# gorse-io/gorse

Measured on AMD Instinct MI355X. Metric: BPR positive-samples/sec (whole job, N GPUs), higher is better.
Workload: dtype f32; 1 GPU; S-ml1m 6040x3706x994169 per rank (C2), nFactors=64; factors_finite=True

## Files before the change

### gorse_amd/csrc/bpr.hip

```cpp
#include <algorithm>
#include <cstdlib>
#include <cstring>

#include "bpr_bins.hpp"
#include "mf_internal.hpp"
#include <utility>

using namespace gorse;

namespace {

int g_variant = 0;
constexpr int MODE_ATOMIC = GORSE_BPR_HOGWILD_ATOMIC;
constexpr int MODE_EXACT = GORSE_BPR_SEQUENTIAL;
constexpr int MODE_RACY = GORSE_BPR_HOGWILD_RACY;
constexpr int MODE_STORES = GORSE_BPR_HOGWILD_STORES;

__global__ __launch_bounds__(256) void bpr_sample_kernel(int32_t U, int32_t I, const int64_t *__restrict__ uptr,
                                                         const int32_t *__restrict__ uidx,
                                                         const int32_t *__restrict__ usorted, uint64_t seed,
                                                         uint64_t epoch, int64_t sample_base, int64_t n,
                                                         int32_t *__restrict__ us, int32_t *__restrict__ is,
                                                         int32_t *__restrict__ js, int32_t *__restrict__ fail_count) {
    for (int64_t s = (int64_t)blockIdx.x * blockDim.x + threadIdx.x; s < n; s += (int64_t)gridDim.x * blockDim.x) {
// ... 549 lines not shown
        }
        __syncthreads();
        if (!big) {
            for (int k = wid; k < ub; k += kFinThreads / 64) {
                const int32_t beg = k ? cnt[k - 1] : 0, len = cnt[k] - beg;
                const uint32_t salt = group_salt(ulo + k);
                if (group && len >= 3 && len <= kGroupCap && ulo + k < U) wave_sort_run(key + beg, len, lane);
                for (int t = lane; t < len; t += 64) {
                    const int2 v = group_unkey(key[beg + t], salt);
                    key[beg + t] = ((uint64_t)(uint32_t)v.y << 32) | (uint32_t)v.x;
                }
            }
            __syncthreads();
        }
        for (int p = tid; p < ms; p += kFinThreads) {
            si[b0 + s0 + p] = (int32_t)(uint32_t)key[p];
            sj[b0 + s0 + p] = (int32_t)(key[p] >> 32);
        }
        __syncthreads();
    }
    if (tid == 0 && nfail > 0) atomicAdd(fail_count, nfail);
    if (big && group)
        for (int k = 0; k < ub && ulo + k < U; k++) {
            const int32_t beg = k ? cnt[k - 1] : 0, len = cnt[k] - beg;
            if (len >= 3 && len <= kGroupCap) group_run<kFinThreads>(key, b0 + beg, len, group_salt(ulo + k), si, sj);
        }
}

template <int MODE>
__device__ __forceinline__ float load_row(const float *p) {
    if (MODE == MODE_EXACT)
        return *p;
    else
        return __hip_atomic_load(p, __ATOMIC_RELAXED, __HIP_MEMORY_SCOPE_AGENT);
}
template <int MODE>
__device__ __forceinline__ void apply(float *p, float snap, float t, float lr, bool fused) {
    if constexpr (MODE == MODE_ATOMIC) {
        (void)snap;
        (void)fused;
        __hip_atomic_fetch_add(p, t * lr, __ATOMIC_RELAXED, __HIP_MEMORY_SCOPE_AGENT);
    } else {
        float r = fused ? fmaf(t, lr, snap) : t * lr + snap;
        if constexpr (MODE == MODE_EXACT)
            *p = r;
        else
            __hip_atomic_store(p, r, __ATOMIC_RELAXED, __HIP_MEMORY_SCOPE_AGENT);
    }
}

__device__ __forceinline__ float bpr_exp(float x, int exp_mode) {
    return exp_mode == 1 ? exp_restated(x) : (exp_mode == 2 ? __expf(x) : expf(x));
}

template <int MODE>
__device__ __forceinline__ void update_elem(float *pu, float *qi, float *qj, int e, float p, float a, float b, float grad,
                                            float nreg, float lr, bool fused, bool same_item) {
    float t1 = p * grad;
    t1 = fused ? fmaf(a, nreg, t1) : a * nreg + t1;
    float t2 = p * (-grad);
    t2 = fused ? fmaf(b, nreg, t2) : b * nreg + t2;
    float t3 = a - b;
    t3 = t3 * grad;
    t3 = fused ? fmaf(p, nreg, t3) : p * nreg + t3;
    if constexpr (MODE == MODE_EXACT) {
        float qi_new = fused ? fmaf(t1, lr, a) : t1 * lr + a;
        qi[e] = qi_new;
        float base = same_item ? qi_new : b;
        qj[e] = fused ? fmaf(t2, lr, base) : t2 * lr + base;
        pu[e] = fused ? fmaf(t3, lr, p) : t3 * lr + p;
    } else {
        apply<MODE>(qi + e, a, t1, lr, fused);
        apply<MODE>(qj + e, b, t2, lr, fused);
        apply<MODE>(pu + e, p, t3, lr, fused);
    }
}

constexpr int kHotReplicas = GORSE_HOT_REPLICAS;
constexpr int kFolderBlocks = 32;
constexpr int kFolderBlocksAcc = 32;
constexpr int kDefaultAccFoldEvery = 4;
int g_acc_fold_every = kDefaultAccFoldEvery;
constexpr uint32_t kDefaultFoldPeriod = 800;
uint32_t g_fold_period = kDefaultFoldPeriod;
constexpr uint64_t kFolderTimeout = 1000000000ull;

struct HotRows {
    const int32_t *slot;
    const int32_t *items;
    const int32_t *meta;
    float *rep;
    int32_t *done;
    int n_hot;
    int d;
    int set;
    uint32_t period;
    int n_acc;
    int acc_every;
};

__device__ __forceinline__ float *hot_row(const HotRows &hot, int32_t code, int64_t group) {
    return hot.rep + (hot_base(code) + (group & ((1 << hot_lg(code)) - 1))) * hot.d;
}

constexpr int kDoneStripes = GORSE_HOT_DONE_STRIPES, kDoneStride = GORSE_HOT_DONE_STRIDE;
constexpr int kFoldPassesWord = 2 * kDoneStripes * kDoneStride;
__device__ __forceinline__ int32_t *done_set(const HotRows &hot, int set) { return hot.done + set * kDoneStripes * kDoneStride; }
template <bool LAST>
__device__ __forceinline__ void worker_done(const HotRows &hot) {
    if constexpr (LAST) asm volatile("s_waitcnt vmcnt(0)" ::: "memory");
    __syncthreads();
    if (threadIdx.x == 0) {
        if constexpr (LAST) {
            __builtin_amdgcn_fence(__ATOMIC_RELEASE, "agent");
            asm volatile("s_waitcnt vmcnt(0)" ::: "memory");
        }
        __hip_atomic_fetch_add(done_set(hot, hot.set) + (blockIdx.x & (kDoneStripes - 1)) * kDoneStride, 1, __ATOMIC_RELAXED,
                               __HIP_MEMORY_SCOPE_AGENT);
    }
}
__device__ __forceinline__ bool workers_done(const HotRows &hot, int workers) {
    const int lane = threadIdx.x & 63;
    const int32_t *c = done_set(hot, hot.set);
    int v = lane < kDoneStripes ? __hip_atomic_load(c + lane * kDoneStride, __ATOMIC_RELAXED, __HIP_MEMORY_SCOPE_AGENT) : 0;
#pragma unroll
    for (int o = 32; o > 0; o >>= 1) v += __shfl_xor(v, o, 64);
    return v >= workers;
}

__device__ __forceinline__ void fold_pass(const HotRows &hot, float *Q, int s0, int s1, int64_t tid, int64_t nthreads) {
    const int d = hot.d;
    const int64_t work = (int64_t)(s1 - s0) * d;
    for (int64_t w = tid; w < work; w += nthreads) {
        const int64_t slot = s0 + w / d;
        const int e = (int)(w - (slot - s0) * d);
        const int32_t code = hot.meta[slot];
        const int nr = 1 << hot_lg(code);
        float *r0 = hot.rep + hot_base(code) * d + e;
        float v[kHotReplicas];
#pragma unroll
        for (int r = 0; r < kHotReplicas; r++)
            v[r] = r < nr ? __hip_atomic_exchange(r0 + (int64_t)r * d, 0.0f, __ATOMIC_RELAXED, __HIP_MEMORY_SCOPE_AGENT) : 0.0f;
        float sum = 0.0f;
#pragma unroll
        for (int r = 0; r < kHotReplicas; r++) sum += v[r];
        if (sum != 0.0f)
            __hip_atomic_fetch_add(Q + (int64_t)hot.items[slot] * d + e, sum, __ATOMIC_RELAXED, __HIP_MEMORY_SCOPE_AGENT);
    }
}

constexpr int kAccBatch = 4;
__device__ __forceinline__ void fold_acc_pass(const HotRows &hot, float *Q, int s0, int s1, int tid, int nthreads) {
    const int d = hot.d;
    const int work = (s1 - s0) * d;
    for (int wb = tid; wb < work; wb += kAccBatch * nthreads) {
        float v[kAccBatch];
        float *q[kAccBatch];
#pragma unroll
        for (int b = 0; b < kAccBatch; b++) {
            const int w = wb + b * nthreads;
            v[b] = 0.0f;
            q[b] = Q;
            if (w < work) {
                const int slot = s0 + w / d;
                const int e = w - (slot - s0) * d;
                q[b] = Q + (int64_t)hot.items[slot] * d + e;
                v[b] = __hip_atomic_exchange(hot.rep + hot_base(hot.meta[slot]) * d + e, 0.0f, __ATOMIC_RELAXED, __HIP_MEMORY_SCOPE_AGENT);
// ... 179 lines not shown
    for (int64_t t0 = 0; t0 < nt; t0 += 256) {
        const int64_t t = t0 + threadIdx.x;
        const int32_t v = t < nt ? sums[t] : 0;
        int32_t total;
        const int32_t ex = block_exclusive_scan_256(v, lds, &total);
        if (t < nt) sums[t] = carry + ex;
        carry += total;
    }
}

__global__ __launch_bounds__(256) void scan_apply_kernel(int32_t *__restrict__ data, int64_t m,
                                                         const int32_t *__restrict__ sums) {
    __shared__ int32_t lds[4];
    const int64_t base = (int64_t)blockIdx.x * kScanTile + (int64_t)threadIdx.x * 8;
    int32_t x[8], v = 0;
#pragma unroll
    for (int e = 0; e < 8; e++) {
        x[e] = base + e < m ? data[base + e] : 0;
        v += x[e];
    }
    int32_t run = sums[blockIdx.x] + block_exclusive_scan_256(v, lds, nullptr);
#pragma unroll
    for (int e = 0; e < 8; e++) {
        if (base + e < m) data[base + e] = run;
        run += x[e];
    }
}


__global__ __launch_bounds__(256) void bpr_scatter_by_kernel(const int32_t *__restrict__ key, const int32_t *__restrict__ us,
                                                             const int32_t *__restrict__ is, const int32_t *__restrict__ js,
                                                             int64_t n, int32_t K, const int32_t *__restrict__ bucket,
                                                             const int32_t *__restrict__ rank, int32_t *__restrict__ su,
                                                             int32_t *__restrict__ si, int32_t *__restrict__ sj) {
    for (int64_t s = (int64_t)blockIdx.x * blockDim.x + threadIdx.x; s < n; s += (int64_t)gridDim.x * blockDim.x) {
        const int32_t kk = key[s] < 0 ? K : key[s];
        const int64_t pos = (int64_t)bucket[kk] + rank[s];
        su[pos] = us[s];
        si[pos] = is[s];
        sj[pos] = js[s];
    }
}

constexpr int kCold = -2;
constexpr int kSeriesFlush = 8;
#ifndef GORSE_BPR_SERIES_SKIP_GATHERS
#define GORSE_BPR_SERIES_SKIP_GATHERS 1
#endif

#ifndef GORSE_BPR_D8_PAIRS
#define GORSE_BPR_D8_PAIRS 1
#endif
template <int NC, bool NEG_STORE, bool D8 = false>
__global__ __launch_bounds__(kBlock) void bpr_update_user_kernel(float *P, float *Q, const int32_t *__restrict__ si,
                                                                 const int32_t *__restrict__ sj,
                                                                 const int32_t *__restrict__ off, int32_t U, int d,
                                                                 float lr, float reg, int exp_mode, double *loss,
                                                                 HotRows hot, int folders, int neg_replicas) {
    if ((int)blockIdx.x < folders) {
        run_folders<true>(hot, Q, folders);
        return;
    }
    auto continues = [](int i0, int j0, int i1, int j1) { return i0 == i1 && (i0 | j0 | j1) >= 0 && i0 != j0 && i0 != j1; };
    const int glane = threadIdx.x & (kGroup - 1);
    const int lane = D8 ? (glane & 7) : glane;
    constexpr int SUBS = D8 && GORSE_BPR_D8_PAIRS ? 2 : 1;
    const bool writer = !D8 || SUBS == 2 || glane < 8;
    auto mad = [](float x, float y, float z) { return D8 ? x * y + z : fmaf(x, y, z); };
    auto tree8 = [](float v) { return SUBS == 2 ? group_tree8_halves(v) : group_tree8(v); };
    const int gib = threadIdx.x / kGroup;
    const int64_t group = ((int64_t)((int)blockIdx.x - folders) * kGroupsPerBlock + gib) * SUBS + (SUBS == 2 ? glane >> 3 : 0);
    const int64_t ngroups = (int64_t)((int)gridDim.x - folders) * kGroupsPerBlock * SUBS;
    const float nreg = -reg;
    double my_loss = 0.0;
    const bool open = folders > 0;
    const bool look_i = open;
    const bool look_j = (open && neg_replicas) || NEG_STORE;
    const int32_t *slot_of = (look_i || look_j) ? hot.slot : si;
    int im1 = -1, jm1 = -1, im2 = -1, jm2 = -1;
    for (int64_t u = group; u < U; u += ngroups) {
        const int beg = off[u], end = off[u + 1];
        if (beg >= end) continue;
        float *pu = P + u * d;
        constexpr int G = 2, IA = 3;
        constexpr int GB = NEG_STORE ? 1 : G;
        float p[NC], ra[G][NC], rb[GB][NC];
        const int last = end - 1;
        auto at = [&](int s) { return s <= last ? s : last; };
        auto cl = [](int x) { return x < 0 ? 0 : x; };
        auto idx_i = [&](int i_, int j_) { return look_i ? cl(i_) : (look_j ? cl(j_) : beg); };
        auto idx_j = [&](int i_, int j_) { return look_j ? cl(j_) : (look_i ? cl(i_) : beg); };
        int ii[IA], jj[IA], sli[G], slj[G];
#pragma unroll
        for (int k = 0; k < IA; k++) ii[k] = si[at(beg + k)], jj[k] = sj[at(beg + k)];
#pragma unroll
        for (int k = 0; k < G; k++) sli[k] = slot_of[idx_i(ii[k], jj[k])], slj[k] = slot_of[idx_j(ii[k], jj[k])];
        float cur[NC], acc[NC];
        bool cont = false;
        int pending = 0;
#pragma unroll
        for (int c = 0; c < NC; c++) {
            p[c] = load_row<MODE_ATOMIC>(pu + 16 * c + lane);
#pragma unroll
            for (int k = 0; k < G; k++) ra[k][c] = load_row<MODE_ATOMIC>(Q + (int64_t)cl(ii[k]) * d + 16 * c + lane);
#pragma unroll
            for (int k = 0; k < GB; k++) rb[k][c] = load_row<MODE_ATOMIC>(Q + (int64_t)cl(jj[k]) * d + 16 * c + lane);
        }
        for (int s = beg; s < end; s++) {
            const int in_ = si[at(s + IA)], jn_ = sj[at(s + IA)];
            const int sli_n = slot_of[idx_i(ii[G], jj[G])];
            const int slj_n = slot_of[idx_j(ii[G], jj[G])];
            const int i = ii[0], j = jj[0], slot = sli[0], slotj = slj[0];
            float(&a)[NC] = ra[0];
            float(&b)[NC] = rb[0];
            float ran[NC], rbn[NC];
            const bool gather_i = !GORSE_BPR_SERIES_SKIP_GATHERS || !(s + G <= last && continues(ii[G - 1], jj[G - 1], ii[G], jj[G]));
#pragma unroll
            for (int c = 0; c < NC; c++) ran[c] = 0.0f;
            if (gather_i) {
#pragma unroll
                for (int c = 0; c < NC; c++) ran[c] = load_row<MODE_ATOMIC>(Q + (int64_t)cl(ii[G]) * d + 16 * c + lane);
            }
#pragma unroll
            for (int c = 0; c < NC; c++) rbn[c] = load_row<MODE_ATOMIC>(Q + (int64_t)cl(jj[GB]) * d + 16 * c + lane);
            if (cont) {
#pragma unroll
                for (int c = 0; c < NC; c++) a[c] = cur[c];
            }
            const bool more = s < last && continues(i, j, ii[1], jj[1]);
            const bool valid = j >= 0;
            float *qi = Q + (int64_t)cl(i) * d, *qj = Q + (int64_t)cl(j) * d;
            if (open && slot >= 0) qi = hot_row(hot, slot, group);
            if (open && neg_replicas && slotj >= 0) qj = hot_row(hot, slotj, group);
            bool st_j = false;
            if constexpr (NEG_STORE) {
                const bool own_j = i == j || j == im1 || j == jm1 || j == im2 || j == jm2;
                st_j = slotj == kCold && !own_j;
            }
            const float diff = D8 ? tree8(p[0] * a[0]) - tree8(p[0] * b[0]) : dot512_regs<NC>(p, a) - dot512_regs<NC>(p, b);
            const float ex = bpr_exp(-diff, exp_mode);
            const float grad = ex / (1.0f + ex);
            if (loss && (SUBS == 2 ? (glane & 7) == 0 : glane == 0) && valid) my_loss += (double)log1pf(ex);
            float t1[NC], t2[NC];
#pragma unroll
            for (int c = 0; c < NC; c++) {
                t1[c] = mad(a[c], nreg, p[c] * grad);
                t2[c] = mad(b[c], nreg, p[c] * (-grad));
                const float t3 = mad(p[c], nreg, (a[c] - b[c]) * grad);
                p[c] = valid ? mad(t3, lr, p[c]) : p[c];
            }
            if (valid) {
#pragma unroll
                for (int c = 0; c < NC; c++) {
                    acc[c] = pending > 0 ? acc[c] + t1[c] * lr : t1[c] * lr;
                    cur[c] = mad(t1[c], lr, a[c]);
                }
                if (!more || ++pending >= kSeriesFlush) {
                    pending = 0;
                    if (writer) {
#pragma unroll
                        for (int c = 0; c < NC; c++)
                            __hip_atomic_fetch_add(qi + 16 * c + lane, acc[c], __ATOMIC_RELAXED, __HIP_MEMORY_SCOPE_AGENT);
                    }
                }
            }
            cont = more;
            if (!valid || !writer) {
            } else if (st_j) {
#pragma unroll
                for (int c = 0; c < NC; c++)
                    __hip_atomic_store(qj + 16 * c + lane, mad(t2[c], lr, b[c]), __ATOMIC_RELAXED, __HIP_MEMORY_SCOPE_AGENT);
            } else {
#pragma unroll
                for (int c = 0; c < NC; c++)
                    __hip_atomic_fetch_add(qj + 16 * c + lane, t2[c] * lr, __ATOMIC_RELAXED, __HIP_MEMORY_SCOPE_AGENT);
            }
#pragma unroll
            for (int c = 0; c < NC; c++) {
#pragma unroll
                for (int k = 0; k + 1 < G; k++) ra[k][c] = ra[k + 1][c];
                ra[G - 1][c] = ran[c];
#pragma unroll
                for (int k = 0; k + 1 < GB; k++) rb[k][c] = rb[k + 1][c];
                rb[GB - 1][c] = rbn[c];
            }
            im2 = im1, jm2 = jm1, im1 = i, jm1 = j;
#pragma unroll
            for (int k = 0; k + 1 < IA; k++) ii[k] = ii[k + 1], jj[k] = jj[k + 1];
            ii[IA - 1] = in_, jj[IA - 1] = jn_;
#pragma unroll
            for (int k = 0; k + 1 < G; k++) sli[k] = sli[k + 1], slj[k] = slj[k + 1];
            sli[G - 1] = sli_n, slj[G - 1] = slj_n;
        }
        if (writer) {
#pragma unroll
            for (int c = 0; c < NC; c++)
                __hip_atomic_store(pu + 16 * c + lane, p[c], __ATOMIC_RELAXED, __HIP_MEMORY_SCOPE_AGENT);
        }
    }
    if (loss && (SUBS == 2 ? (glane & 7) == 0 : glane == 0) && my_loss != 0.0) atomicAdd(loss, my_loss);
    if (folders > 0) worker_done<true>(hot);
}

__global__ __launch_bounds__(256) void scan_small_kernel(int32_t *__restrict__ data, int64_t m) {
    __shared__ int32_t lds[4];
    int32_t carry = 0;
    for (int64_t t0 = 0; t0 < m; t0 += kScanTile) {
        const int64_t base = t0 + (int64_t)threadIdx.x * 8;
        int32_t x[8], v = 0;
#pragma unroll
        for (int e = 0; e < 8; e++) {
            x[e] = base + e < m ? data[base + e] : 0;
            v += x[e];
        }
        int32_t total;
        int32_t run = carry + block_exclusive_scan_256(v, lds, &total);
#pragma unroll
        for (int e = 0; e < 8; e++) {
            if (base + e < m) data[base + e] = run;
            run += x[e];
        }
        carry += total;
    }
}

int32_t exclusive_scan_i32(int32_t *data, int64_t m, int32_t *tmp, hipStream_t st) {
    const int64_t nt = ceil_div(m, kScanTile);
    if (nt <= 16) {
        scan_small_kernel<<<dim3(1), dim3(256), 0, st>>>(data, m);
        GORSE_HIP_CHECK(hipGetLastError());
        return GORSE_OK;
    }
    scan_tile_sums_kernel<<<dim3((unsigned)nt), dim3(256), 0, st>>>(data, m, tmp);
    scan_sums_kernel<<<dim3(1), dim3(256), 0, st>>>(tmp, nt);
    scan_apply_kernel<<<dim3((unsigned)nt), dim3(256), 0, st>>>(data, m, tmp);
    GORSE_HIP_CHECK(hipGetLastError());
    return GORSE_OK;
}


int32_t launch_user_sort(gorse_mf *h, const int32_t *trip, int32_t *sorted, int32_t *bucket, int32_t *rank, int64_t n, size_t cap,
                         hipStream_t st) {
    const int64_t m = h->U + 2;
    const int64_t blocks = std::min<int64_t>(ceil_div(n, 256), 256 * 8);
    GORSE_HIP_CHECK(hipMemsetAsync(bucket, 0, (size_t)m * sizeof(int32_t), st));
    if (g_variant & GORSE_TEST_BPR_STABLE_RANK)
        bpr_rank_kernel<<<dim3(1), dim3(1), 0, st>>>(trip, n, (int32_t)h->U, bucket, rank);
    else
        bpr_rank_kernel<<<dim3((unsigned)blocks), dim3(256), 0, st>>>(trip, n, (int32_t)h->U, bucket, rank);
    GORSE_TRY(exclusive_scan_i32(bucket, m, h->scan_tmp2.p, st));
    bpr_scatter_by_kernel<<<dim3((unsigned)blocks), dim3(256), 0, st>>>(trip, trip, trip + cap, trip + 2 * cap, n,
                                                                       (int32_t)h->U, bucket, rank, sorted,
                                                                       sorted + cap, sorted + 2 * cap);
    GORSE_HIP_CHECK(hipGetLastError());
    return GORSE_OK;
}
int32_t ensure_user_sort(gorse_mf *h) {
    const int64_t m = h->U + 2;
    const size_t mat = prep_matrix_words(h->U, (int64_t)h->trip_cap);
    if ((size_t)m <= h->ubucket[0].n && h->scan_tmp2.n >= (size_t)ceil_div(m, kScanTile) && h->urank[0].n >= 2 * h->trip_cap &&
        h->ubins.n >= (size_t)2 * kMaxBins && h->ubinmat.n >= mat)
        return GORSE_OK;
    GORSE_TRY(mf_sync_streams(h));
    if (h->ubins.n < (size_t)2 * kMaxBins) GORSE_TRY(h->ubins.alloc((size_t)2 * kMaxBins));
    if (h->ubinmat.n < mat) GORSE_TRY(h->ubinmat.alloc(mat));
    for (int b = 0; b < 2; b++) {
        GORSE_TRY(h->ubucket[b].alloc((size_t)m));
        GORSE_TRY(h->urank[b].alloc(2 * h->trip_cap));
    }
    if (h->scan_tmp2.n < (size_t)ceil_div(m, kScanTile)) GORSE_TRY(h->scan_tmp2.alloc((size_t)ceil_div(m, kScanTile)));
    return GORSE_OK;
}
bool user_runs_supported(const gorse_mf *h) {
    return (h->d == 8 || h->d == 16 || h->d == 32 || h->d == 64 || h->d == 128) && (h->U >= 4096 || (g_variant & GORSE_TEST_BPR_USER_RUNS));
}

constexpr int kDefaultStoreMode = 1;
int g_store_mode = kDefaultStoreMode;

HotRows make_hot(const gorse_mf *h) {
    return HotRows{h->hot_slot.p, h->hot_items.p, h->hot_meta.p, h->hot_rep.p, h->hot_done.p, 0, h->d, 0, g_fold_period, 0, g_acc_fold_every};
}
bool has_hot(const gorse_mf *h) { return h->n_hot > 0 || h->n_acc > 0; }
int open_hot(gorse_mf *h, HotRows &hot) {
    hot.n_hot = h->n_hot;
    hot.n_acc = h->n_acc;
    hot.set = (int)(h->hot_launches++ & 1);
    return kFolderBlocks + (h->n_acc > 0 ? kFolderBlocksAcc : 0);
}

int32_t launch_update_users(gorse_mf *h, const int32_t *sorted, const int32_t *bucket, size_t cap, float lr, float reg,
                            int exp_mode, double *loss, hipStream_t st, bool stores, hipEvent_t start = nullptr,
                            hipEvent_t stop = nullptr) {
    const int d = h->d;
    int64_t blocks = ceil_div(h->U, (int64_t)kGroupsPerBlock * (d == 8 && GORSE_BPR_D8_PAIRS ? 2 : 1));
    const int64_t capb = 256 * 16;
    if (blocks > capb) blocks = capb;
    HotRows hot = make_hot(h);
    const int folders = has_hot(h) ? open_hot(h, hot) : 0;
    blocks += folders;
    const int neg_rep = hot.n_acc > 0 || (hot.n_hot > 0 && hot_neg_replicas(hot.n_hot, h->I)) ? 1 : 0;
    dim3 grid((unsigned)blocks), block(kBlock);
    const bool neg_store = stores && h->n_cold > 0 && g_store_mode == 1;
#define LAUNCH2(NC, NEG_STORE)                                                                                         \
    hipExtLaunchKernelGGL((bpr_update_user_kernel<(NC == 0 ? 1 : NC), NEG_STORE, NC == 0>), grid, block, 0, st, start, stop, 0,     \
                          h->P.p, h->Q.p, sorted + cap, sorted + 2 * cap, bucket, (int32_t)h->U, d, lr, reg, exp_mode, loss, hot, \
                          folders, neg_rep)
#define LAUNCH(NC)                                                                                                     \
    do {                                                                                                               \
        if (neg_store)                                                                                                 \
            LAUNCH2(NC, true);                                                                                         \
        else                                                                                                           \
            LAUNCH2(NC, false);                                                                                        \
    } while (0)
    if (d == 8)
        LAUNCH(0);
    else if (d == 16)
        LAUNCH(1);
    else if (d == 32)
        LAUNCH(2);
    else if (d == 64)
        LAUNCH(4);
    else
        LAUNCH(8);
#undef LAUNCH2
#undef LAUNCH
    GORSE_HIP_CHECK(hipGetLastError());
    return GORSE_OK;
}

template <int MODE>
int32_t launch_update_mode(gorse_mf *h, const int32_t *us, const int32_t *is, const int32_t *js, const int32_t *order,
                           int64_t begin, int64_t end, float lr, float reg, int exp_mode, double *loss,
                           hipStream_t st, hipEvent_t start, hipEvent_t stop) {
    const int64_t n = end - begin;
    if (n <= 0) return GORSE_OK;
    const int d = h->d;
    int64_t blocks = ceil_div(n, kGroupsPerBlock);
    const int64_t cap = 256 * 16;
    if (blocks > cap) blocks = cap;
    HotRows hot = make_hot(h);
    const int folders = MODE == MODE_ATOMIC && has_hot(h) ? open_hot(h, hot) : 0;
    blocks += folders;
    dim3 grid((unsigned)blocks), block(kBlock);
#define LAUNCH(NC, SH)                                                                                               \
    hipExtLaunchKernelGGL((bpr_update_kernel<NC, MODE>), grid, block, SH, st, start, folders > 0 ? nullptr : stop, 0, h->P.p, \
                          h->Q.p, us, is, js, order, begin, end, d, lr, reg, exp_mode, loss, hot, folders)
    if (d == 16)
        LAUNCH(1, 0);
    else if (d == 32)
        LAUNCH(2, 0);
    else if (d == 64)
        LAUNCH(4, 0);
    else if (d == 128)
        LAUNCH(8, 0);
    else
        LAUNCH(0, (size_t)kGroupsPerBlock * 3 * d * sizeof(float));
#undef LAUNCH
    GORSE_HIP_CHECK(hipGetLastError());
    if (folders > 0) {
        const int64_t fb = std::min<int64_t>(ceil_div((int64_t)(hot.n_hot + hot.n_acc) * d, 256), 512);
        hipExtLaunchKernelGGL(bpr_fold_kernel, dim3((unsigned)fb), dim3(256), 0, st, nullptr, stop, 0, hot, h->Q.p);
        GORSE_HIP_CHECK(hipGetLastError());
    }
    return GORSE_OK;
}

int32_t launch_update(gorse_mf *h, int mode, const int32_t *us, const int32_t *is, const int32_t *js,
                      const int32_t *order, int64_t begin, int64_t end, float lr, float reg, int exp_mode, double *loss,
                      hipStream_t st, hipEvent_t start = nullptr, hipEvent_t stop = nullptr) {
    switch (mode) {
    case MODE_ATOMIC:
        return launch_update_mode<MODE_ATOMIC>(h, us, is, js, order, begin, end, lr, reg, exp_mode, loss, st, start, stop);
    case MODE_EXACT:
        return launch_update_mode<MODE_EXACT>(h, us, is, js, order, begin, end, lr, reg, exp_mode, loss, st, start, stop);
    case MODE_RACY:
        return launch_update_mode<MODE_RACY>(h, us, is, js, order, begin, end, lr, reg, exp_mode, loss, st, start, stop);
    }
    return fail(GORSE_ERR_INVALID, "unknown BPR mode %d", mode);
}

// ... 196 lines not shown
        if (uruns) GORSE_TRY(ensure_user_sort(h));
        int64_t c = 0;
        for (int64_t s0 = 0; s0 < n_samples; s0 += cap, c++) {
            const int b = (int)(h->chunk_seq & 1);
            h->chunk_seq++;
            const int64_t m = std::min(cap, n_samples - s0);
            if (cancel && *cancel) {
                GORSE_TRY(mf_sync_streams(h));
                return fail(GORSE_ERR_CANCELLED, "cancelled");
            }
            int32_t *tb = h->trip[b].p;
            const hipStream_t prep = h->stream2;
            if (h->ev_consumed[b]) GORSE_HIP_CHECK(hipStreamWaitEvent(prep, h->ev_consumed[b], 0));
            if (uruns && !stable_rank) {
                GORSE_TRY(launch_prepare_users(h, seed, epoch, base + s0, m, tb, h->sorted[b].p, h->ubucket[b].p, h->urank[b].p,
                                               (size_t)cap, prep));
            } else {
                hipEvent_t sa = nullptr, sb = nullptr;
                h->prof.events(GORSE_PROF_BPR_SAMPLE, &sa, &sb);
                GORSE_TRY(launch_sampler(h, seed, epoch, base + s0, m, tb, (size_t)cap, prep, sa, sb));
            }
            GORSE_HIP_CHECK(hipEventRecord(h->ev_sampled[b], prep));
            GORSE_HIP_CHECK(hipStreamWaitEvent(h->stream, h->ev_sampled[b], 0));
            if (stable_rank) {
                const int tok = h->prof.begin(GORSE_PROF_BPR_SORT, h->stream);
                GORSE_TRY(launch_user_sort(h, tb, h->sorted[b].p, h->ubucket[b].p, h->urank[b].p, m, (size_t)cap, h->stream));
                h->prof.end(tok, h->stream);
            }
            hipEvent_t start = nullptr, stop = nullptr;
            h->prof.events(GORSE_PROF_BPR_UPDATE, &start, &stop);
            const bool last = s0 + cap >= n_samples;
            if (!start && c == 0) start = ep_begin;
            if (!stop) stop = last ? mf_epoch_end_event(h) : h->ev_chunk[(h->chunk_seq - 1) % gorse_mf::kChunkRing];
            if (uruns)
                GORSE_TRY(launch_update_users(h, h->sorted[b].p, h->ubucket[b].p, (size_t)cap, lr, reg, g_exp_mode_exact, d_loss, h->stream,
                                              mode == MODE_STORES, start, stop));
            else
                GORSE_TRY(launch_update(h, mode == MODE_STORES ? MODE_ATOMIC : mode, tb, tb + cap, tb + 2 * cap, nullptr, 0, m, lr, reg, 0, d_loss,
                                        h->stream, start, stop));
            h->ev_consumed[b] = stop;
            if (last) ep_end = stop;
            if (cancel && (c & 7) == 7) GORSE_TRY(mf_sync_streams(h));
        }
    }
    GORSE_TRY(mf_epoch_end(h, ep_end));
    h->ep_chain = true;
    if (sync || loss_out) {
        if (loss_out)
            GORSE_HIP_CHECK(hipMemcpyAsync(loss_out, h->loss.p, sizeof(double), hipMemcpyDeviceToHost, h->stream));
        GORSE_TRY(mf_sync_streams(h));
        GORSE_TRY(mf_epoch_harvest(h, true));
    }
    return GORSE_OK;
}

}

extern "C" void gorse_hip_test_set_exact_exp(int32_t mode) { g_exp_mode_exact = mode; }

extern "C" int32_t gorse_mf_bpr_schedule(gorse_mf *h, int32_t *user_runs) {
    if (!h || !user_runs) return fail(GORSE_ERR_INVALID, "NULL argument");
    *user_runs = (user_runs_enabled() && user_runs_supported(h)) ? 1 : 0;
    return GORSE_OK;
}
extern "C" void gorse_hip_test_set_variant(int32_t v) {
    g_variant = v & (GORSE_TEST_BPR_USER_RUNS | GORSE_TEST_BPR_PER_SAMPLE | GORSE_TEST_BPR_STABLE_RANK | GORSE_TEST_BPR_THREE_KERNELS |
                     GORSE_TEST_BPR_ARRIVAL_ORDER | GORSE_TEST_BPR_NO_BINS);
}
extern "C" void gorse_hip_test_set_bpr_chunk(int64_t samples) { g_chunk_override = samples; }
extern "C" int32_t gorse_hip_test_bpr_fail_count(gorse_mf *h, int32_t *count) {
    if (!h || !count) return fail(GORSE_ERR_INVALID, "NULL argument");
    GORSE_TRY(h->use());
    GORSE_TRY(mf_sync_streams(h));
    GORSE_HIP_CHECK(hipMemcpy(count, h->fail_count.p, sizeof(int32_t), hipMemcpyDeviceToHost));
    return GORSE_OK;
}
extern "C" void gorse_hip_test_bpr_finish_capacities(int32_t *samples, int32_t *row_entries) {
    if (samples) *samples = kFinCap;
    if (row_entries) *row_entries = kFinStage;
}
extern "C" void gorse_hip_test_set_bpr_store_mode(int32_t store_mode) {
    g_store_mode = store_mode < 0 ? kDefaultStoreMode : (store_mode & 1);
}
extern "C" void gorse_hip_test_set_bpr_fold_period(int32_t ticks) { g_fold_period = ticks > 0 ? (uint32_t)ticks : kDefaultFoldPeriod; }
extern "C" void gorse_hip_test_set_bpr_acc_fold_every(int32_t periods) { g_acc_fold_every = periods > 0 ? periods : kDefaultAccFoldEvery; }
extern "C" int32_t gorse_hip_test_bpr_fold_stats(gorse_mf *h, int64_t *out3) {
    if (!h || !out3) return fail(GORSE_ERR_INVALID, "NULL argument");
    GORSE_TRY(h->use());
    GORSE_TRY(mf_sync_streams(h));
    int32_t passes = 0;
    if (h->hot_done.p)
        GORSE_HIP_CHECK(hipMemcpy(&passes, h->hot_done.p + kFoldPassesWord, sizeof(int32_t), hipMemcpyDeviceToHost));
    out3[0] = passes, out3[1] = h->n_hot, out3[2] = h->hot_rows;
    return GORSE_OK;
}
extern "C" int32_t gorse_hip_test_bpr_hot_state(gorse_mf *h, int32_t *items, int32_t *replicas, float *rep) {
    if (!h) return fail(GORSE_ERR_INVALID, "handle is NULL");
    GORSE_TRY(h->use());
    GORSE_TRY(mf_sync_streams(h));
    const size_t n = (size_t)h->n_hot;
    std::vector<int32_t> meta(n);
    if (n > 0) {
        if (items) GORSE_HIP_CHECK(hipMemcpy(items, h->hot_items.p, n * sizeof(int32_t), hipMemcpyDeviceToHost));
        GORSE_HIP_CHECK(hipMemcpy(meta.data(), h->hot_meta.p, n * sizeof(int32_t), hipMemcpyDeviceToHost));
    }
    if (replicas)
        for (size_t s = 0; s < n; s++) replicas[s] = 1 << hot_lg(meta[s]);
    if (rep && h->hot_rows > 0)
        GORSE_HIP_CHECK(hipMemcpy(rep, h->hot_rep.p, (size_t)h->hot_rows * h->d * sizeof(float), hipMemcpyDeviceToHost));
    return GORSE_OK;
}

extern "C" int32_t gorse_hip_test_bpr_acc_state(gorse_mf *h, int32_t *items, float *rows) {
    if (!h) return fail(GORSE_ERR_INVALID, "handle is NULL");
    GORSE_TRY(h->use());
    GORSE_TRY(mf_sync_streams(h));
    const size_t n = (size_t)h->n_acc;
    if (n == 0) return GORSE_OK;
    if (items) GORSE_HIP_CHECK(hipMemcpy(items, h->hot_items.p + h->n_hot, n * sizeof(int32_t), hipMemcpyDeviceToHost));
    if (rows)
        GORSE_HIP_CHECK(hipMemcpy(rows, h->hot_rep.p + (size_t)h->hot_rows * h->d, n * h->d * sizeof(float), hipMemcpyDeviceToHost));
    return GORSE_OK;
}
extern "C" int32_t gorse_hip_test_bpr_item_classes(gorse_mf *h, int32_t *slot, int64_t *out2) {
    if (!h) return fail(GORSE_ERR_INVALID, "handle is NULL");
    GORSE_TRY(h->use());
    GORSE_TRY(mf_sync_streams(h));
    if (slot && h->hot_slot.p) GORSE_HIP_CHECK(hipMemcpy(slot, h->hot_slot.p, (size_t)h->I * sizeof(int32_t), hipMemcpyDeviceToHost));
    if (out2) out2[0] = h->n_acc, out2[1] = h->n_cold;
    return GORSE_OK;
}

extern "C" int32_t gorse_bpr_epoch(gorse_mf *h, int64_t n_samples, float lr, float reg, uint64_t seed, uint64_t epoch,
                                   int64_t sample_base, int32_t mode, const volatile int32_t *cancel, double *loss_out) {
    return epoch_impl(h, n_samples, lr, reg, seed, epoch, sample_base, mode, cancel, loss_out, true);
}

extern "C" int32_t gorse_bpr_epoch_enqueue(gorse_mf *h, int64_t n_samples, float lr, float reg, uint64_t seed,
                                           uint64_t epoch, int64_t sample_base, int32_t mode) {
    if (mode == MODE_EXACT) return fail(GORSE_ERR_INVALID, "the sequential schedule cannot be enqueued asynchronously");
    return epoch_impl(h, n_samples, lr, reg, seed, epoch, sample_base, mode, nullptr, nullptr, false);
}

extern "C" int32_t gorse_bpr_sample_triplets(gorse_mf *h, int64_t n, uint64_t seed, uint64_t epoch, int64_t sample_base,
                                             int32_t *u, int32_t *i, int32_t *j) {
    if (!h) return fail(GORSE_ERR_INVALID, "handle is NULL");
    if (n < 0 || (n > 0 && (!u || !i || !j))) return fail(GORSE_ERR_INVALID, "bad arguments");
    if (n == 0) return GORSE_OK;
    GORSE_TRY(h->use());
    GORSE_TRY(ensure_trip(h, n));
    GORSE_TRY(mf_sync_streams(h));
    const int64_t cap = (int64_t)h->trip_cap;
    for (int64_t s0 = 0; s0 < n; s0 += cap) {
        const int64_t m = std::min(cap, n - s0);
        int32_t *tb = h->trip[0].p;
        GORSE_TRY(launch_sampler(h, seed, epoch, sample_base + s0, m, tb, (size_t)cap, h->stream));
        GORSE_HIP_CHECK(hipMemcpyAsync(u + s0, tb, (size_t)m * 4, hipMemcpyDeviceToHost, h->stream));
        GORSE_HIP_CHECK(hipMemcpyAsync(i + s0, tb + cap, (size_t)m * 4, hipMemcpyDeviceToHost, h->stream));
        GORSE_HIP_CHECK(hipMemcpyAsync(j + s0, tb + 2 * cap, (size_t)m * 4, hipMemcpyDeviceToHost, h->stream));
        GORSE_HIP_CHECK(hipStreamSynchronize(h->stream));
    }
    return GORSE_OK;
}

extern "C" int32_t gorse_hip_test_bpr_prepare_chunk(gorse_mf *h, int64_t n, uint64_t seed, uint64_t epoch, int64_t sample_base,
                                                    int32_t *off , int32_t *si , int32_t *sj ) {
    if (!h || !off || !si || !sj) return fail(GORSE_ERR_INVALID, "NULL argument");
// ... 52 lines not shown
```

Measured before the change: 2.518 billion samples/s.

## Use register ring buffer for BPR user-run prefetch and tune fold period per d

Replaces the shift-register prefetch pipeline in the user-run BPR kernel with a ring buffer of depth 4, indexed by compile-time phases inside an unrolled loop. This removes the per-sample register shuffling of prefetched Q rows and indices and deepens the index lookahead. It also makes the hot-row fold period depend on factor count, using shorter periods for d=8 and d=16 in user-run mode. The costs are more VGPRs per thread, which can lower occupancy, and a masked tail phase for partial ring iterations.

```diff
diff --git a/gorse_amd/csrc/bpr.hip b/gorse_amd/csrc/bpr.hip
--- a/gorse_amd/csrc/bpr.hip
+++ b/gorse_amd/csrc/bpr.hip
@@ -655,7 +655,12 @@
 constexpr int kDefaultAccFoldEvery = 4;
 int g_acc_fold_every = kDefaultAccFoldEvery;
 constexpr uint32_t kDefaultFoldPeriod = 800;
-uint32_t g_fold_period = kDefaultFoldPeriod;
+uint32_t g_fold_period = 0;
+uint32_t fold_period_of(int d, bool user_runs) {
+    if (g_fold_period) return g_fold_period;
+    if (user_runs && d == 8) return 300;
+    return user_runs && d == 16 ? kDefaultFoldPeriod / 2 : kDefaultFoldPeriod;
+}
 constexpr uint64_t kFolderTimeout = 1000000000ull;
 
 struct HotRows {
@@ -1001,115 +1006,222 @@
         const int beg = off[u], end = off[u + 1];
         if (beg >= end) continue;
         float *pu = P + u * d;
-        constexpr int G = 2, IA = 3;
-        constexpr int GB = NEG_STORE ? 1 : G;
-        float p[NC], ra[G][NC], rb[GB][NC];
-        const int last = end - 1;
-        auto at = [&](int s) { return s <= last ? s : last; };
-        auto cl = [](int x) { return x < 0 ? 0 : x; };
-        auto idx_i = [&](int i_, int j_) { return look_i ? cl(i_) : (look_j ? cl(j_) : beg); };
-        auto idx_j = [&](int i_, int j_) { return look_j ? cl(j_) : (look_i ? cl(i_) : beg); };
-        int ii[IA], jj[IA], sli[G], slj[G];
-#pragma unroll
-        for (int k = 0; k < IA; k++) ii[k] = si[at(beg + k)], jj[k] = sj[at(beg + k)];
-#pragma unroll
-        for (int k = 0; k < G; k++) sli[k] = slot_of[idx_i(ii[k], jj[k])], slj[k] = slot_of[idx_j(ii[k], jj[k])];
-        float cur[NC], acc[NC];
-        bool cont = false;
-        int pending = 0;
-#pragma unroll
-        for (int c = 0; c < NC; c++) {
-            p[c] = load_row<MODE_ATOMIC>(pu + 16 * c + lane);
-#pragma unroll
-            for (int k = 0; k < G; k++) ra[k][c] = load_row<MODE_ATOMIC>(Q + (int64_t)cl(ii[k]) * d + 16 * c + lane);
-#pragma unroll
-            for (int k = 0; k < GB; k++) rb[k][c] = load_row<MODE_ATOMIC>(Q + (int64_t)cl(jj[k]) * d + 16 * c + lane);
-        }
-        for (int s = beg; s < end; s++) {
-            const int in_ = si[at(s + IA)], jn_ = sj[at(s + IA)];
-            const int sli_n = slot_of[idx_i(ii[G], jj[G])];
-            const int slj_n = slot_of[idx_j(ii[G], jj[G])];
-            const int i = ii[0], j = jj[0], slot = sli[0], slotj = slj[0];
-            float(&a)[NC] = ra[0];
-            float(&b)[NC] = rb[0];
-            float ran[NC], rbn[NC];
-            const bool gather_i = !GORSE_BPR_SERIES_SKIP_GATHERS || !(s + G <= last && continues(ii[G - 1], jj[G - 1], ii[G], jj[G]));
-#pragma unroll
-            for (int c = 0; c < NC; c++) ran[c] = 0.0f;
-            if (gather_i) {
-#pragma unroll
-                for (int c = 0; c < NC; c++) ran[c] = load_row<MODE_ATOMIC>(Q + (int64_t)cl(ii[G]) * d + 16 * c + lane);
-            }
-#pragma unroll
-            for (int c = 0; c < NC; c++) rbn[c] = load_row<MODE_ATOMIC>(Q + (int64_t)cl(jj[GB]) * d + 16 * c + lane);
-            if (cont) {
-#pragma unroll
-                for (int c = 0; c < NC; c++) a[c] = cur[c];
-            }
-            const bool more = s < last && continues(i, j, ii[1], jj[1]);
-            const bool valid = j >= 0;
-            float *qi = Q + (int64_t)cl(i) * d, *qj = Q + (int64_t)cl(j) * d;
-            if (open && slot >= 0) qi = hot_row(hot, slot, group);
-            if (open && neg_replicas && slotj >= 0) qj = hot_row(hot, slotj, group);
-            bool st_j = false;
-            if constexpr (NEG_STORE) {
-                const bool own_j = i == j || j == im1 || j == jm1 || j == im2 || j == jm2;
-                st_j = slotj == kCold && !own_j;
-            }
-            const float diff = D8 ? tree8(p[0] * a[0]) - tree8(p[0] * b[0]) : dot512_regs<NC>(p, a) - dot512_regs<NC>(p, b);
-            const float ex = bpr_exp(-diff, exp_mode);
-            const float grad = ex / (1.0f + ex);
-            if (loss && (SUBS == 2 ? (glane & 7) == 0 : glane == 0) && valid) my_loss += (double)log1pf(ex);
-            float t1[NC], t2[NC];
-#pragma unroll
+        constexpr bool kRing = !(NC == 8 && NEG_STORE);
+        float p[NC];
+        if constexpr (kRing) {
+            constexpr int G = 2, IA = 4, R = 4;
+            static_assert(R % G == 0 && IA <= R && G < IA, "ring positions are compile-time phase numbers");
+            constexpr int GB = NEG_STORE ? 1 : G;
+            float ra[R][NC], rb[R][NC];
+            const int last = end - 1;
+            auto at = [&](int s) { return s <= last ? s : last; };
+            auto cl = [](int x) { return x < 0 ? 0 : x; };
+            auto idx_i = [&](int i_, int j_) { return look_i ? cl(i_) : (look_j ? cl(j_) : beg); };
+            auto idx_j = [&](int i_, int j_) { return look_j ? cl(j_) : (look_i ? cl(i_) : beg); };
+            int ii[R], jj[R], sli[R], slj[R];
+    #pragma unroll
+            for (int k = 0; k < IA; k++) ii[k] = si[at(beg + k)], jj[k] = sj[at(beg + k)];
+    #pragma unroll
+            for (int k = 0; k < G; k++) sli[k] = slot_of[idx_i(ii[k], jj[k])], slj[k] = slot_of[idx_j(ii[k], jj[k])];
+            float cur[NC], acc[NC];
+            bool cont = false;
+            int pending = 0;
+    #pragma unroll
             for (int c = 0; c < NC; c++) {
-                t1[c] = mad(a[c], nreg, p[c] * grad);
-                t2[c] = mad(b[c], nreg, p[c] * (-grad));
-                const float t3 = mad(p[c], nreg, (a[c] - b[c]) * grad);
-                p[c] = valid ? mad(t3, lr, p[c]) : p[c];
-            }
-            if (valid) {
-#pragma unroll
+                p[c] = load_row<MODE_ATOMIC>(pu + 16 * c + lane);
+    #pragma unroll
+                for (int k = 0; k < G; k++) ra[k][c] = load_row<MODE_ATOMIC>(Q + (int64_t)cl(ii[k]) * d + 16 * c + lane);
+    #pragma unroll
+                for (int k = 0; k < GB; k++) rb[k][c] = load_row<MODE_ATOMIC>(Q + (int64_t)cl(jj[k]) * d + 16 * c + lane);
+            }
+            for (int s0 = beg; s0 <= last; s0 += R) {
+    #pragma unroll
+                for (int ph = 0; ph < R; ph++) {
+                    const int s = s0 + ph;
+                    const bool act = s <= last;
+                    constexpr int kMask = R - 1;
+                    const int r0 = ph, r1 = (ph + 1) & kMask, rg1 = (ph + G - 1) & kMask, rg = (ph + G) & kMask, rn = (ph + IA) & kMask;
+                    int i, j;
+                    asm volatile("v_mov_b32 %0, %1" : "=v"(i) : "v"(ii[r0]));
+                    asm volatile("v_mov_b32 %0, %1" : "=v"(j) : "v"(jj[r0]));
+                    ii[rn] = si[at(s + IA)], jj[rn] = sj[at(s + IA)];
+                    sli[rg] = slot_of[idx_i(ii[rg], jj[rg])];
+                    slj[rg] = slot_of[idx_j(ii[rg], jj[rg])];
+                    const bool gather_i = !GORSE_BPR_SERIES_SKIP_GATHERS || !(s + G <= last && continues(ii[rg1], jj[rg1], ii[rg], jj[rg]));
+                    if (gather_i) {
+    #pragma unroll
+                        for (int c = 0; c < NC; c++) ra[rg][c] = load_row<MODE_ATOMIC>(Q + (int64_t)cl(ii[rg]) * d + 16 * c + lane);
+                    }
+    #pragma unroll
+                    for (int c = 0; c < NC; c++)
+                        rb[(ph + GB) & kMask][c] = load_row<MODE_ATOMIC>(Q + (int64_t)cl(jj[(ph + GB) & kMask]) * d + 16 * c + lane);
+                    const int slot = sli[r0], slotj = slj[r0];
+                    float a[NC];
+                    float(&b)[NC] = rb[r0];
+    #pragma unroll
+                    for (int c = 0; c < NC; c++) a[c] = cont ? cur[c] : ra[r0][c];
+                    const bool more = s < last && continues(i, j, ii[r1], jj[r1]);
+                    const bool valid = j >= 0 && act;
+                    float *qi = Q + (int64_t)cl(i) * d, *qj = Q + (int64_t)cl(j) * d;
+                    if (open && slot >= 0) qi = hot_row(hot, slot, group);
+                    if (open && neg_replicas && slotj >= 0) qj = hot_row(hot, slotj, group);
+                    bool st_j = false;
+                    if constexpr (NEG_STORE) {
+                        const bool own_j = i == j || j == im1 || j == jm1 || j == im2 || j == jm2;
+                        st_j = slotj == kCold && !own_j;
+                    }
+                    const float diff = D8 ? tree8(p[0] * a[0]) - tree8(p[0] * b[0]) : dot512_regs<NC>(p, a) - dot512_regs<NC>(p, b);
+                    const float ex = bpr_exp(-diff, exp_mode);
+                    const float grad = ex / (1.0f + ex);
+                    if (loss && (SUBS == 2 ? (glane & 7) == 0 : glane == 0) && valid) my_loss += (double)log1pf(ex);
+                    float t1[NC], t2[NC];
+    #pragma unroll
+                    for (int c = 0; c < NC; c++) {
+                        t1[c] = mad(a[c], nreg, p[c] * grad);
+                        t2[c] = mad(b[c], nreg, p[c] * (-grad));
+                        const float t3 = mad(p[c], nreg, (a[c] - b[c]) * grad);
+                        p[c] = valid ? mad(t3, lr, p[c]) : p[c];
+                    }
+                    if (valid) {
+    #pragma unroll
+                        for (int c = 0; c < NC; c++) {
+                            acc[c] = pending > 0 ? acc[c] + t1[c] * lr : t1[c] * lr;
+                            cur[c] = mad(t1[c], lr, a[c]);
+                        }
+                        if (!more || ++pending >= kSeriesFlush) {
+                            pending = 0;
+                            if (writer) {
+    #pragma unroll
+                                for (int c = 0; c < NC; c++)
+                                    __hip_atomic_fetch_add(qi + 16 * c + lane, acc[c], __ATOMIC_RELAXED, __HIP_MEMORY_SCOPE_AGENT);
+                            }
+                        }
+                    }
+                    if (act) cont = more;
+                    if (!valid || !writer) {
+                    } else if (st_j) {
+    #pragma unroll
+                        for (int c = 0; c < NC; c++)
+                            __hip_atomic_store(qj + 16 * c + lane, mad(t2[c], lr, b[c]), __ATOMIC_RELAXED, __HIP_MEMORY_SCOPE_AGENT);
+                    } else {
+    #pragma unroll
+                        for (int c = 0; c < NC; c++)
+                            __hip_atomic_fetch_add(qj + 16 * c + lane, t2[c] * lr, __ATOMIC_RELAXED, __HIP_MEMORY_SCOPE_AGENT);
+                    }
+                    if (act) im2 = im1, jm2 = jm1, im1 = i, jm1 = j;
+                }
+            }
+        } else {
+            constexpr int G = 2, IA = 3;
+            constexpr int GB = NEG_STORE ? 1 : G;
+            float ra[G][NC], rb[GB][NC];
+            const int last = end - 1;
+            auto at = [&](int s) { return s <= last ? s : last; };
+            auto cl = [](int x) { return x < 0 ? 0 : x; };
+            auto idx_i = [&](int i_, int j_) { return look_i ? cl(i_) : (look_j ? cl(j_) : beg); };
+            auto idx_j = [&](int i_, int j_) { return look_j ? cl(j_) : (look_i ? cl(i_) : beg); };
+            int ii[IA], jj[IA], sli[G], slj[G];
+    #pragma unroll
+            for (int k = 0; k < IA; k++) ii[k] = si[at(beg + k)], jj[k] = sj[at(beg + k)];
+    #pragma unroll
+            for (int k = 0; k < G; k++) sli[k] = slot_of[idx_i(ii[k], jj[k])], slj[k] = slot_of[idx_j(ii[k], jj[k])];
+            float cur[NC], acc[NC];
+            bool cont = false;
+            int pending = 0;
+    #pragma unroll
+            for (int c = 0; c < NC; c++) {
+                p[c] = load_row<MODE_ATOMIC>(pu + 16 * c + lane);
+    #pragma unroll
+                for (int k = 0; k < G; k++) ra[k][c] = load_row<MODE_ATOMIC>(Q + (int64_t)cl(ii[k]) * d + 16 * c + lane);
+    #pragma unroll
+                for (int k = 0; k < GB; k++) rb[k][c] = load_row<MODE_ATOMIC>(Q + (int64_t)cl(jj[k]) * d + 16 * c + lane);
+            }
+            for (int s = beg; s < end; s++) {
+                const int in_ = si[at(s + IA)], jn_ = sj[at(s + IA)];
+                const int sli_n = slot_of[idx_i(ii[G], jj[G])];
+                const int slj_n = slot_of[idx_j(ii[G], jj[G])];
+                const int i = ii[0], j = jj[0], slot = sli[0], slotj = slj[0];
+                float(&a)[NC] = ra[0];
+                float(&b)[NC] = rb[0];
+                float ran[NC], rbn[NC];
+                const bool gather_i = !GORSE_BPR_SERIES_SKIP_GATHERS || !(s + G <= last && continues(ii[G - 1], jj[G - 1], ii[G], jj[G]));
+    #pragma unroll
+                for (int c = 0; c < NC; c++) ran[c] = 0.0f;
+                if (gather_i) {
+    #pragma unroll
+                    for (int c = 0; c < NC; c++) ran[c] = load_row<MODE_ATOMIC>(Q + (int64_t)cl(ii[G]) * d + 16 * c + lane);
+                }
+    #pragma unroll
+                for (int c = 0; c < NC; c++) rbn[c] = load_row<MODE_ATOMIC>(Q + (int64_t)cl(jj[GB]) * d + 16 * c + lane);
+                if (cont) {
+    #pragma unroll
+                    for (int c = 0; c < NC; c++) a[c] = cur[c];
+                }
+                const bool more = s < last && continues(i, j, ii[1], jj[1]);
+                const bool valid = j >= 0;
+                float *qi = Q + (int64_t)cl(i) * d, *qj = Q + (int64_t)cl(j) * d;
+                if (open && slot >= 0) qi = hot_row(hot, slot, group);
+                if (open && neg_replicas && slotj >= 0) qj = hot_row(hot, slotj, group);
+                bool st_j = false;
+                if constexpr (NEG_STORE) {
+                    const bool own_j = i == j || j == im1 || j == jm1 || j == im2 || j == jm2;
+                    st_j = slotj == kCold && !own_j;
+                }
+                const float diff = D8 ? tree8(p[0] * a[0]) - tree8(p[0] * b[0]) : dot512_regs<NC>(p, a) - dot512_regs<NC>(p, b);
+                const float ex = bpr_exp(-diff, exp_mode);
+                const float grad = ex / (1.0f + ex);
+                if (loss && (SUBS == 2 ? (glane & 7) == 0 : glane == 0) && valid) my_loss += (double)log1pf(ex);
+                float t1[NC], t2[NC];
+    #pragma unroll
                 for (int c = 0; c < NC; c++) {
-                    acc[c] = pending > 0 ? acc[c] + t1[c] * lr : t1[c] * lr;
-                    cur[c] = mad(t1[c], lr, a[c]);
+                    t1[c] = mad(a[c], nreg, p[c] * grad);
+                    t2[c] = mad(b[c], nreg, p[c] * (-grad));
+                    const float t3 = mad(p[c], nreg, (a[c] - b[c]) * grad);
+                    p[c] = valid ? mad(t3, lr, p[c]) : p[c];
                 }
-                if (!more || ++pending >= kSeriesFlush) {
-                    pending = 0;
-                    if (writer) {
-#pragma unroll
-                        for (int c = 0; c < NC; c++)
-                            __hip_atomic_fetch_add(qi + 16 * c + lane, acc[c], __ATOMIC_RELAXED, __HIP_MEMORY_SCOPE_AGENT);
+                if (valid) {
+    #pragma unroll
+                    for (int c = 0; c < NC; c++) {
+                        acc[c] = pending > 0 ? acc[c] + t1[c] * lr : t1[c] * lr;
+                        cur[c] = mad(t1[c], lr, a[c]);
+                    }
+                    if (!more || ++pending >= kSeriesFlush) {
+                        pending = 0;
+                        if (writer) {
+    #pragma unroll
+                            for (int c = 0; c < NC; c++)
+                                __hip_atomic_fetch_add(qi + 16 * c + lane, acc[c], __ATOMIC_RELAXED, __HIP_MEMORY_SCOPE_AGENT);
+                        }
                     }
                 }
-            }
-            cont = more;
-            if (!valid || !writer) {
-            } else if (st_j) {
-#pragma unroll
-                for (int c = 0; c < NC; c++)
-                    __hip_atomic_store(qj + 16 * c + lane, mad(t2[c], lr, b[c]), __ATOMIC_RELAXED, __HIP_MEMORY_SCOPE_AGENT);
-            } else {
-#pragma unroll
-                for (int c = 0; c < NC; c++)
-                    __hip_atomic_fetch_add(qj + 16 * c + lane, t2[c] * lr, __ATOMIC_RELAXED, __HIP_MEMORY_SCOPE_AGENT);
-            }
-#pragma unroll
-            for (int c = 0; c < NC; c++) {
-#pragma unroll
-                for (int k = 0; k + 1 < G; k++) ra[k][c] = ra[k + 1][c];
-                ra[G - 1][c] = ran[c];
-#pragma unroll
-                for (int k = 0; k + 1 < GB; k++) rb[k][c] = rb[k + 1][c];
-                rb[GB - 1][c] = rbn[c];
-            }
-            im2 = im1, jm2 = jm1, im1 = i, jm1 = j;
-#pragma unroll
-            for (int k = 0; k + 1 < IA; k++) ii[k] = ii[k + 1], jj[k] = jj[k + 1];
-            ii[IA - 1] = in_, jj[IA - 1] = jn_;
-#pragma unroll
-            for (int k = 0; k + 1 < G; k++) sli[k] = sli[k + 1], slj[k] = slj[k + 1];
-            sli[G - 1] = sli_n, slj[G - 1] = slj_n;
+                cont = more;
+                if (!valid || !writer) {
+                } else if (st_j) {
+    #pragma unroll
+                    for (int c = 0; c < NC; c++)
+                        __hip_atomic_store(qj + 16 * c + lane, mad(t2[c], lr, b[c]), __ATOMIC_RELAXED, __HIP_MEMORY_SCOPE_AGENT);
+                } else {
+    #pragma unroll
+                    for (int c = 0; c < NC; c++)
+                        __hip_atomic_fetch_add(qj + 16 * c + lane, t2[c] * lr, __ATOMIC_RELAXED, __HIP_MEMORY_SCOPE_AGENT);
+                }
+    #pragma unroll
+                for (int c = 0; c < NC; c++) {
+    #pragma unroll
+                    for (int k = 0; k + 1 < G; k++) ra[k][c] = ra[k + 1][c];
+                    ra[G - 1][c] = ran[c];
+    #pragma unroll
+                    for (int k = 0; k + 1 < GB; k++) rb[k][c] = rb[k + 1][c];
+                    rb[GB - 1][c] = rbn[c];
+                }
+                im2 = im1, jm2 = jm1, im1 = i, jm1 = j;
+    #pragma unroll
+                for (int k = 0; k + 1 < IA; k++) ii[k] = ii[k + 1], jj[k] = jj[k + 1];
+                ii[IA - 1] = in_, jj[IA - 1] = jn_;
+    #pragma unroll
+                for (int k = 0; k + 1 < G; k++) sli[k] = sli[k + 1], slj[k] = slj[k + 1];
+                sli[G - 1] = sli_n, slj[G - 1] = slj_n;
+            }
         }
         if (writer) {
 #pragma unroll
@@ -1198,7 +1310,7 @@
 int g_store_mode = kDefaultStoreMode;
 
 HotRows make_hot(const gorse_mf *h) {
-    return HotRows{h->hot_slot.p, h->hot_items.p, h->hot_meta.p, h->hot_rep.p, h->hot_done.p, 0, h->d, 0, g_fold_period, 0, g_acc_fold_every};
+    return HotRows{h->hot_slot.p, h->hot_items.p, h->hot_meta.p, h->hot_rep.p, h->hot_done.p, 0, h->d, 0, fold_period_of(h->d, false), 0, g_acc_fold_every};
 }
 bool has_hot(const gorse_mf *h) { return h->n_hot > 0 || h->n_acc > 0; }
 int open_hot(gorse_mf *h, HotRows &hot) {
@@ -1216,6 +1328,7 @@
     const int64_t capb = 256 * 16;
     if (blocks > capb) blocks = capb;
     HotRows hot = make_hot(h);
+    hot.period = fold_period_of(d, true);
     const int folders = has_hot(h) ? open_hot(h, hot) : 0;
     blocks += folders;
     const int neg_rep = hot.n_acc > 0 || (hot.n_hot > 0 && hot_neg_replicas(hot.n_hot, h->I)) ? 1 : 0;
@@ -1578,7 +1691,7 @@
 extern "C" void gorse_hip_test_set_bpr_store_mode(int32_t store_mode) {
     g_store_mode = store_mode < 0 ? kDefaultStoreMode : (store_mode & 1);
 }
-extern "C" void gorse_hip_test_set_bpr_fold_period(int32_t ticks) { g_fold_period = ticks > 0 ? (uint32_t)ticks : kDefaultFoldPeriod; }
+extern "C" void gorse_hip_test_set_bpr_fold_period(int32_t ticks) { g_fold_period = ticks > 0 ? (uint32_t)ticks : 0; }
 extern "C" void gorse_hip_test_set_bpr_acc_fold_every(int32_t periods) { g_acc_fold_every = periods > 0 ? periods : kDefaultAccFoldEvery; }
 extern "C" int32_t gorse_hip_test_bpr_fold_stats(gorse_mf *h, int64_t *out3) {
     if (!h || !out3) return fail(GORSE_ERR_INVALID, "NULL argument");
```

Measured after the change: 2.526 billion samples/s (median of 6 runs). Within noise of the previous version (+0.3%).
